# Ighina/MultimodalTopicSegmentation

Hardware: AMD Instinct MI355X
Metric: sentences/sec (fwd+bwd) (higher is better)
Workload: dtype bf16; 1 GPU; BASELINE configs[1]: restricted-window transformer tagger d=1792 heads=8 ff=256 radius=15 layers=1 focal loss, 64 docs x 256 sentences per GPU, fwd+bwd+Adam(eps 1e-7), inputs resident in HBM; global_batch_docs=64, sentences_per_doc=256, parallelism=dp1 (document-sharded, RCCL all-reduce)

## Files before the change

multimodaltopicsegmentation_amd/csrc/gemm.hip:

```cpp
#include <atomic>
#include <algorithm>
#include <math.h>
#include <stdlib.h>
#include "common.h"

#include "gemm_common.h"


template <int LAYOUT, typename TC, bool GLDS>
__global__ __launch_bounds__(256, 2) void gemm_bf16_kernel(const GemmArgs a) {
  constexpr bool A_KMAJOR = (LAYOUT == MTS_NT || LAYOUT == MTS_NN);
  constexpr bool B_KMAJOR = (LAYOUT == MTS_NT || LAYOUT == MTS_TT);
  extern __shared__ __attribute__((aligned(16))) char smem[];

  const int tid = threadIdx.x;
  const int lane = tid & 63;
  const int wave = tid >> 6;
  const int wm = wave >> 1, wn = wave & 1;
  const int r16 = lane & 15, g = lane >> 4;

  const int ntn = (a.N + BN - 1) / BN;
  const int ntm = (a.M + BM - 1) / BM;
  const int nt = ntn * ntm;
  int bid = blockIdx.x;
// ... 488 lines not shown
  const int m = (int)(idx / n4), n = 4 * (int)(idx % n4);
  float s[4] = {0.f, 0.f, 0.f, 0.f};
  if (accumulate) load4<float>(C + (size_t)m * ldc + n, s);
  const size_t plane = (size_t)M * N;
  for (int z = 0; z < splits; ++z) {
    float v[4];
    load4<float>(slab + z * plane + (size_t)m * N + n, v);
#pragma unroll
    for (int i = 0; i < 4; ++i) s[i] += v[i];
  }
  store4<float>(C + (size_t)m * ldc + n, s);
}

__global__ __launch_bounds__(256) void splitk_reduce_t_kernel(const float* __restrict__ slab, int splits, int M, int N, float* __restrict__ Ct,
                                                              int ldc, int accumulate) {
  __shared__ float tile[32][33];
  const int n0 = blockIdx.x * 32, m0 = blockIdx.y * 32;
  const int tx = threadIdx.x & 31, ty = threadIdx.x >> 5;
  const size_t plane = (size_t)M * N;
#pragma unroll
  for (int r = ty; r < 32; r += 8) {
    const int m = m0 + r, n = n0 + tx;
    float s = 0.f;
    if (m < M && n < N) {
      const float* p = slab + (size_t)m * N + n;
      int z = 0;
      for (; z + 7 < splits; z += 8) {
        float v[8];
#pragma unroll
        for (int u = 0; u < 8; ++u) v[u] = p[(size_t)(z + u) * plane];
#pragma unroll
        for (int u = 0; u < 8; ++u) s += v[u];
      }
      for (; z < splits; ++z) s += p[(size_t)z * plane];
    }
    tile[r][tx] = s;
  }
  __syncthreads();
#pragma unroll
  for (int r = ty; r < 32; r += 8) {
    const int n = n0 + r, m = m0 + tx;
    if (n < N && m < M) {
      float* o = Ct + (size_t)n * ldc + m;
      *o = accumulate ? *o + tile[tx][r] : tile[tx][r];
    }
  }
}

template <typename T> __global__ void cast_kernel(const float* __restrict__ src, T* __restrict__ dst, size_t n) {
  size_t i = ((size_t)blockIdx.x * blockDim.x + threadIdx.x) * 4;
  const size_t stride = (size_t)gridDim.x * blockDim.x * 4;
  for (; i + 3 < n; i += stride) {
    float v[4];
    load4<float>(src + i, v);
    store4<T>(dst + i, v);
  }
  if (i < n && i + 3 >= n)
    for (size_t j = i; j < n; ++j) dst[j] = from_f32<T>(src[j]);
}

template <typename T> __global__ void cast_concat_kernel(const float* __restrict__ s1, const float* __restrict__ s2, T* __restrict__ dst,
                                                          size_t rows, int D1, int D2) {
  const int D = D1 + D2, q = D / 4;
  const size_t total = rows * q;
  for (size_t i = (size_t)blockIdx.x * blockDim.x + threadIdx.x; i < total; i += (size_t)gridDim.x * blockDim.x) {
    const size_t r = i / q;
    const int e = (int)(i - r * q) * 4;
    float v[4];
    load4<float>(e < D1 ? s1 + r * D1 + e : s2 + r * D2 + (e - D1), v);
    store4<T>(dst + r * D + e, v);
  }
}

extern "C" int mts_cast_concat(void* stream, int dst_dtype, size_t rows, int D1, int D2, const float* src1, const float* src2, void* dst) {
  MTS_CHECK_ARG(src1 && src2 && dst && D1 > 0 && D2 > 0 && D1 % 4 == 0 && D2 % 4 == 0, "mts_cast_concat: bad arguments (widths must be multiples of 4)");
  if (rows == 0) return MTS_OK;
  const int blocks = (int)std::min<size_t>(4096, (rows * ((D1 + D2) / 4) + 255) / 256);
  if (dst_dtype == MTS_BF16) hipLaunchKernelGGL(cast_concat_kernel<bf16_t>, dim3(blocks), dim3(256), 0, (hipStream_t)stream, src1, src2, (bf16_t*)dst, rows, D1, D2);
  else if (dst_dtype == MTS_F32) hipLaunchKernelGGL(cast_concat_kernel<float>, dim3(blocks), dim3(256), 0, (hipStream_t)stream, src1, src2, (float*)dst, rows, D1, D2);
  else { mts_set_error("mts_cast_concat: bad dtype %d", dst_dtype); return MTS_ERR_INVALID; }
  MTS_LAUNCH_CHECK("mts_cast_concat");
  return MTS_OK;
}

extern "C" size_t mts_colsum_workspace(int N) { return (size_t)COLSUM_RS * (size_t)N * sizeof(float); }

extern "C" int mts_colsum(void* stream, int dtype, int M, int N, const void* X, int ldx, float* out, int accumulate,
                          void* partial) {
  MTS_CHECK_ARG(M > 0 && N > 0 && X && out && partial, "mts_colsum: bad arguments");
  MTS_CHECK_ARG(dtype == MTS_F32 || dtype == MTS_BF16, "mts_colsum: bad dtype %d", dtype);
  MTS_CHECK_ARG(ldx % 4 == 0, "mts_colsum: ldx must be a multiple of 4");
  hipStream_t st = (hipStream_t)stream;
  const int nparts = min(COLSUM_RS, M);
  dim3 grid(ceil_div(N, 64), COLSUM_RS);
  (void)nparts;
  if (dtype == MTS_F32)
    hipLaunchKernelGGL(colsum_partial_kernel<float>, grid, dim3(256), 0, st, (const float*)X, M, N, ldx, (float*)partial);
  else
    hipLaunchKernelGGL(colsum_partial_kernel<bf16_t>, grid, dim3(256), 0, st, (const bf16_t*)X, M, N, ldx, (float*)partial);
  hipLaunchKernelGGL(colsum_final_kernel, dim3(ceil_div(N, 64)), dim3(256), 0, st, (const float*)partial, N, COLSUM_RS, out,
                     accumulate);
  MTS_LAUNCH_CHECK("mts_colsum");
  return MTS_OK;
}

extern "C" int mts_cast(void* stream, int dst_dtype, const float* src, void* dst, size_t n) {
  MTS_CHECK_ARG(src && dst, "mts_cast: null pointer");
  if (n == 0) return MTS_OK;
  hipStream_t st = (hipStream_t)stream;
  const int blocks = (int)std::min<size_t>(2048, (n / 4 + 255) / 256 + 1);
  if (dst_dtype == MTS_BF16)
    hipLaunchKernelGGL(cast_kernel<bf16_t>, dim3(blocks), dim3(256), 0, st, src, (bf16_t*)dst, n);
  else if (dst_dtype == MTS_F32)
    hipLaunchKernelGGL(cast_kernel<float>, dim3(blocks), dim3(256), 0, st, src, (float*)dst, n);
  else {
    mts_set_error("mts_cast: bad dtype %d", dst_dtype);
    return MTS_ERR_INVALID;
  }
  MTS_LAUNCH_CHECK("mts_cast");
  return MTS_OK;
}

int mts_launch_gemm256(const GemmArgs& a, int layout, bool c_is_f32, int splits, hipStream_t st);
int mts_launch_gemm224(const GemmArgs& a, int layout, bool c_is_f32, int splits, hipStream_t st);
bool mts_gemm224t_applies(const GemmArgs& a, int layout, bool c_is_f32, int splits);

static thread_local int g_gemm_glds = -1;
static thread_local int g_tile_mode = -1;
static thread_local int g_force_splits = 0;
static thread_local int g_tile_order = 1;
static thread_local int g_gemm_deep = 1;
static thread_local int g_chain = 0;
static thread_local int g_combine = 0;
#define MTS_GEMM_WS_HEAD 8192
static thread_local int g_last_tile = 0, g_last_splits = 0;

static thread_local void (*g_mid_hook)(void) = nullptr;
extern "C" int mts_gemm_set_mid_hook(void (*fn)(void)) { g_mid_hook = fn; return MTS_OK; }

extern "C" int mts_gemm_last_plan(int* tile, int* splits) {
  if (tile) *tile = g_last_tile;
  if (splits) *splits = g_last_splits;
  return MTS_OK;
}

void mts_band_set_mfma(int on);
void mts_band_set_fused(int on);
static thread_local int g_f32_mfma = 1;
static thread_local int g_big_min_k = 256;
static thread_local int g_gemm_variant = 0;
void mts_lstm_pair_set_spin_limit(int n);
void mts_lstm_pair_set_max_pairs(int n);
void mts_lstm_pair_set_parts(int n);
extern "C" int mts_set_option(const char* key, int value) {
  if (!key) return MTS_ERR_INVALID;
  if (!strcmp(key, "gemm_tile")) { g_tile_mode = value; return MTS_OK; }
  if (!strcmp(key, "gemm_glds")) { g_gemm_glds = value; return MTS_OK; }
  if (!strcmp(key, "gemm_splits")) { g_force_splits = value; return MTS_OK; }
  if (!strcmp(key, "gemm_order")) { g_tile_order = value; return MTS_OK; }
  if (!strcmp(key, "gemm_chain")) { g_chain = value; return MTS_OK; }
  if (!strcmp(key, "gemm_combine")) { g_combine = value; return MTS_OK; }
  if (!strcmp(key, "gemm_deep")) { g_gemm_deep = value; return MTS_OK; }
  if (!strcmp(key, "gemm_variant")) { g_gemm_variant = value; return MTS_OK; }
  if (!strcmp(key, "gemm_big_min_k")) { g_big_min_k = value; return MTS_OK; }
  if (!strcmp(key, "gemm_f32_mfma")) { g_f32_mfma = value; return MTS_OK; }
  if (!strcmp(key, "band_mfma")) { mts_band_set_mfma(value); return MTS_OK; }
  if (!strcmp(key, "band_fused_bwd")) { mts_band_set_fused(value); return MTS_OK; }
  if (!strcmp(key, "lstm_pair_spin_limit")) { mts_lstm_pair_set_spin_limit(value); return MTS_OK; }
  if (!strcmp(key, "lstm_pair_max_pairs")) { mts_lstm_pair_set_max_pairs(value); return MTS_OK; }
  if (!strcmp(key, "lstm_parts")) { mts_lstm_pair_set_parts(value); return MTS_OK; }
  mts_set_error("mts_set_option: unknown key %s", key);
  return MTS_ERR_INVALID;
}

template <int LAYOUT, typename TC>
static void launch_bf16(const GemmArgs& a, int splits, hipStream_t st) {
  const int nt = ceil_div(a.M, BM) * ceil_div(a.N, BN);
  if (g_gemm_glds < 0) {
    const char* e = getenv("MTS_GEMM_GLDS");
    g_gemm_glds = (e && e[0] == '0') ? 0 : 1;
  }
  const bool glds = g_gemm_glds && (a.K % BK == 0) && (a.ksplit % BK == 0) && a.M >= 8 && a.N >= 8;
  if (glds) {
    GemmArgs b = a;
    const bool deep = g_gemm_deep && (size_t)nt * splits <= 256 && a.ksplit >= 4 * BK;
    b.nbuf = deep ? 4 : 2;
    auto k = gemm_bf16_kernel<LAYOUT, TC, true>;
    static std::atomic<bool> attr_set{false};
    if (deep && !attr_set.load(std::memory_order_acquire)) {
      if (hipFuncSetAttribute((const void*)k, hipFuncAttributeMaxDynamicSharedMemorySize, 8 * TILE_BYTES) != hipSuccess) b.nbuf = 2;
      else attr_set.store(true, std::memory_order_release);
    }
    hipLaunchKernelGGL(k, dim3(nt, 1, splits), dim3(256), (b.nbuf == 4 ? 8 : 4) * TILE_BYTES, st, b);
  } else {
    hipLaunchKernelGGL((gemm_bf16_kernel<LAYOUT, TC, false>), dim3(nt, 1, splits), dim3(256), 4 * TILE_BYTES, st, a);
  }
}

static void plan_bf16(int c_dtype, int layout, int M, int N, int K, unsigned epilogue, bool has_workspace, size_t workspace_bytes,
                      int* use256_out, int* splits_out) {
  if (g_tile_mode < 0) {
    const char* e = getenv("MTS_GEMM_TILE");
    g_tile_mode = e ? atoi(e) : 0;
  }
  const int tile_mode = g_tile_mode;
  const unsigned plain = epilogue & ~MTS_EPI_ACCUM;
  const bool can_split = (c_dtype == MTS_F32 && plain == 0 && has_workspace && N % 4 == 0 && K >= 2048);
  const bool can256 = (K % BK == 0) && K >= g_big_min_k && M >= 8 && N >= 8 && tile_mode != 128;
  const double bw = 3500.0;
  double best = 1e30;
  int splits = 1;
  int use256 = 0;
  const bool can224 = can256 && (N % 224 == 0) && tile_mode != 256;
  for (int big = 0; big <= (can256 ? 2 : 0); ++big) {
    if (big == 2 && !can224) continue;
    if (tile_mode == 256 && can256 && big != 1) continue;
    if (tile_mode == 224 && can224 && big != 2) continue;
    const int tile = big ? 256 : 128;
    const double slots = big ? 256.0 : 512.0;
    const double t_k = layout == MTS_TN ? (big == 2 ? (M % 256 == 0 ? 0.0160 : 0.0200) : big == 1 ? 0.0218 : 0.0145)
                                        : (big ? 0.0232 * (big == 2 ? 0.875 : 1.0) : 0.0180);
    const double t_0 = big ? 7.7 : 6.5;
    const int nt = ceil_div(M, tile) * (big == 2 ? N / 224 : ceil_div(N, tile));
    for (int sp = 1; sp <= (can_split ? 32 : 1); ++sp) {
      const int ks = ceil_div(ceil_div(K, sp), BK) * BK;
      if (ceil_div(K, ks) != sp) continue;
      if (sp > 1 && (size_t)sp * M * N * sizeof(float) > workspace_bytes) break;
      if (g_force_splits > 0 && can_split && sp != g_force_splits) continue;
      const double rounds = ceil((double)nt * sp / slots);
      const double cost = rounds * (ks * t_k + t_0) + (sp > 1 ? (2.0 * sp + 1.0) * M * N * 4.0 / 1e6 / bw : 0.0);
      if (cost < best) { best = cost; splits = sp; use256 = big; }
    }
  }
  *use256_out = use256;
  *splits_out = splits;
}

int mts_gemm224_last_kernel();
int mts_launch_gemm224t_pair(const GemmArgs& a, int splits, const void* A2, const void* B2, float* slab2, hipStream_t st);
bool mts_gemm224t_applies(const GemmArgs& a, int layout, bool c_is_f32, int splits);

static int wgrad_pair_splits(int M, int N, int K, size_t workspace_bytes) {
  if (M % 256 || N % 224 || K % 64 || K < 256) return -1;
  static int cus = 0;
  if (!cus) { int dev = 0; hipDeviceProp_t pr; cus = (hipGetDevice(&dev) == hipSuccess && hipGetDeviceProperties(&pr, dev) == hipSuccess) ? pr.multiProcessorCount : 256; }
  const int nt = (M / 256) * (N / 224);
  int sp = std::max(1, std::min(32, cus / (2 * nt)));
  for (; sp >= 1; --sp) {
    const int ks = ceil_div(ceil_div(K, sp), BK) * BK;
    if (ceil_div(K, ks) != sp) continue;
    if (ks >= 128 && K - (sp - 1) * ks >= 128 && (size_t)2 * sp * M * N * sizeof(float) <= workspace_bytes) return sp;
  }
  return -1;
}
extern "C" size_t mts_wgrad_pair_workspace(int M, int N, int K) {
  const int sp = wgrad_pair_splits(M, N, K, (size_t)-1);
  return sp < 1 ? 0 : (size_t)2 * sp * M * N * sizeof(float);
}
extern "C" int mts_wgrad_pair(void* stream, int M, int N, int K, const void* A1, const void* B1, float* C1, int ldc1, const void* A2, const void* B2,
                              float* C2t, int ldc2t, int lda, int ldb, int accumulate, void* workspace, size_t workspace_bytes) {
  MTS_CHECK_ARG(M > 0 && N > 0 && K > 0 && A1 && B1 && C1 && A2 && B2 && C2t && workspace, "mts_wgrad_pair: bad arguments");
  MTS_CHECK_ARG(ldc1 >= N && ldc2t >= M && ldc1 % 4 == 0, "mts_wgrad_pair: bad output strides");
  const int sp = wgrad_pair_splits(M, N, K, workspace_bytes);
  MTS_UNSUPPORTED(sp >= 1, "mts_wgrad_pair: M=%d N=%d K=%d not covered (M %% 256, N %% 224, K %% 64) or workspace too small", M, N, K);
  hipStream_t st = (hipStream_t)stream;
  GemmArgs a;
  memset(&a, 0, sizeof(a));
  a.A = A1; a.B = B1; a.C = C1;
  a.M = M; a.N = N; a.K = K; a.lda = lda; a.ldb = ldb; a.ldc = ldc1;
  a.epi = 0; a.colscale = 1.0f;
  a.ksplit = ceil_div(ceil_div(K, sp), BK) * BK;
  a.order = 1; a.nbuf = 2; a.variant = 0;
  float* const planes = (float*)workspace;
  a.slab = planes;
  float* const planes2 = planes + (size_t)sp * M * N;
  MTS_UNSUPPORTED(mts_gemm224t_applies(a, MTS_TN, true, sp), "mts_wgrad_pair: operands not covered by the four-wave weight-gradient kernel (alignment / strides)");
  const int rc = mts_launch_gemm224t_pair(a, sp, A2, B2, planes2, st);
  MTS_UNSUPPORTED(rc == MTS_OK, "mts_wgrad_pair: launch refused");
  hipLaunchKernelGGL(splitk_reduce_kernel, dim3((unsigned)(((size_t)M * (N / 4) + 255) / 256)), dim3(256), 0, st, (const float*)planes, sp, M, N, C1, ldc1,
                     accumulate ? 1 : 0);
  hipLaunchKernelGGL(splitk_reduce_t_kernel, dim3(ceil_div(N, 32), ceil_div(M, 32)), dim3(256), 0, st, (const float*)planes2, sp, M, N, C2t, ldc2t,
                     accumulate ? 1 : 0);
  MTS_LAUNCH_CHECK("mts_wgrad_pair");
  return MTS_OK;
}

extern "C" int mts_gemm_plan(int a_dtype, int c_dtype, int layout, int M, int N, int K, unsigned epilogue, size_t workspace_bytes,
                             int* tile, int* splits) {
  MTS_CHECK_ARG(M > 0 && N > 0 && K > 0, "mts_gemm_plan: bad shape M=%d N=%d K=%d", M, N, K);
  MTS_CHECK_ARG(layout == MTS_NT || layout == MTS_NN || layout == MTS_TN || layout == MTS_TT, "mts_gemm_plan: bad layout %d", layout);
  MTS_CHECK_ARG(a_dtype == MTS_F32 || a_dtype == MTS_BF16, "mts_gemm_plan: bad a_dtype %d", a_dtype);
  int use256 = 0, sp = 1;
  const size_t ws_planes = workspace_bytes > MTS_GEMM_WS_HEAD ? workspace_bytes - MTS_GEMM_WS_HEAD : 0;
  if (a_dtype == MTS_BF16) plan_bf16(c_dtype, layout, M, N, K, epilogue, ws_planes > 0, ws_planes, &use256, &sp);
  if (tile) *tile = a_dtype == MTS_F32 ? (g_f32_mfma ? 128 : 64) : use256 == 2 ? 224 : use256 == 1 ? 256 : 128;
  if (splits) *splits = sp;
  return MTS_OK;
}

extern "C" int mts_gemm(void* stream, int a_dtype, int c_dtype, int layout, int M, int N, int K, const void* A, int lda,
                        const void* B, int ldb, void* C, int ldc, const float* bias, const void* residual, int ldr,
                        void* aux, int ldaux, unsigned epilogue, float colscale, int ncols_scaled, void* workspace, size_t workspace_bytes) {
  MTS_CHECK_ARG(M > 0 && N > 0 && K > 0, "mts_gemm: bad shape M=%d N=%d K=%d", M, N, K);
  MTS_CHECK_ARG(A && B && C, "mts_gemm: null operand");
  MTS_CHECK_ARG(layout == MTS_NT || layout == MTS_NN || layout == MTS_TN || layout == MTS_TT, "mts_gemm: bad layout %d", layout);
  MTS_CHECK_ARG(a_dtype == MTS_F32 || a_dtype == MTS_BF16, "mts_gemm: bad a_dtype %d", a_dtype);
  MTS_CHECK_ARG(c_dtype == MTS_F32 || c_dtype == a_dtype, "mts_gemm: c_dtype must be f32 or a_dtype");
  MTS_CHECK_ARG(!(epilogue & MTS_EPI_BIAS) || bias, "mts_gemm: MTS_EPI_BIAS without bias");
  MTS_CHECK_ARG(!(epilogue & MTS_EPI_RESIDUAL) || residual, "mts_gemm: MTS_EPI_RESIDUAL without residual");
  MTS_CHECK_ARG(!(epilogue & MTS_EPI_ACCUM) || c_dtype == MTS_F32, "mts_gemm: MTS_EPI_ACCUM needs fp32 C");
  MTS_CHECK_ARG((epilogue & (MTS_EPI_GELU | MTS_EPI_RELU)) != (MTS_EPI_GELU | MTS_EPI_RELU), "mts_gemm: MTS_EPI_GELU and MTS_EPI_RELU are exclusive");
  hipStream_t st = (hipStream_t)stream;
  GemmArgs a;
  a.A = A; a.B = B; a.C = C; a.bias = bias; a.residual = residual; a.aux = aux;
  a.M = M; a.N = N; a.K = K; a.lda = lda; a.ldb = ldb; a.ldc = ldc; a.ldr = ldr; a.ldaux = ldaux;
  a.epi = epilogue; a.colscale = colscale; a.ncols_scaled = ncols_scaled;
  a.variant = g_gemm_variant;
#ifdef MTS_GEMM_STAMPS
  a.stamps = nullptr;
#endif
  a.ksplit = K; a.slab = nullptr; a.chain = nullptr; a.order = g_tile_order; a.nbuf = 2;

  if (a_dtype == MTS_F32) {
// ... 87 lines not shown
```

multimodaltopicsegmentation_amd/csrc/norm.hip:

```cpp
#include <algorithm>
#include <type_traits>
#include "common.h"
#include "loss_elems.h"

#define ROW_WAVES 4
#define BWD_MAX_BLOCKS 512

template <typename T, int NV> struct RowRegs {
  float v[NV][4];
  __device__ __forceinline__ void load(const T* row, int D, int lane) {
#pragma unroll
    for (int i = 0; i < NV; ++i) {
      const int e = 4 * (lane + 64 * i);
      if (e < D) load4<T>(row + e, v[i]);
      else { v[i][0] = v[i][1] = v[i][2] = v[i][3] = 0.f; }
    }
  }
  __device__ __forceinline__ void store(T* row, int D, int lane) const {
#pragma unroll
    for (int i = 0; i < NV; ++i) {
      const int e = 4 * (lane + 64 * i);
      if (e < D) store4<T>(row + e, v[i]);
    }
  }
  __device__ __forceinline__ void zero() {
#pragma unroll
    for (int i = 0; i < NV; ++i) v[i][0] = v[i][1] = v[i][2] = v[i][3] = 0.f;
  }
};

template <int NV> __device__ __forceinline__ void row_stats(const float (&x)[NV][4], int D, int lane, float& mean, float& rstd, float eps) {
  float s = 0.f;
#pragma unroll
  for (int i = 0; i < NV; ++i) s += (x[i][0] + x[i][1]) + (x[i][2] + x[i][3]);
  mean = wave_sum(s) / (float)D;
  float q = 0.f;
#pragma unroll
  for (int i = 0; i < NV; ++i) {
    if (4 * (lane + 64 * i) < D) {
#pragma unroll
      for (int j = 0; j < 4; ++j) { const float d = x[i][j] - mean; q += d * d; }
    }
  }
  rstd = 1.0f / sqrtf(wave_sum(q) / (float)D + eps);
}

template <typename T, int NV, int EMBED, bool FULL = false>
__global__ __launch_bounds__(64 * ROW_WAVES) void ln_fwd_kernel(
    const void* __restrict__ xin, const float* __restrict__ pos, int pos_offset, int L, const float* __restrict__ type0,
    const float* __restrict__ gamma, const float* __restrict__ beta, float eps, int rows, int D,
    T* __restrict__ y, T* __restrict__ pre, float* __restrict__ mean_out, float* __restrict__ rstd_out,
    const float* __restrict__ head_w, const float* __restrict__ head_b, int n_out, float* __restrict__ scores,
    const int32_t* __restrict__ row_src, const float* __restrict__ xin2 = nullptr, int D1 = 0) {
  const int lane = threadIdx.x & 63;
  const int row = blockIdx.x * ROW_WAVES + (threadIdx.x >> 6);
  if (row >= rows) return;
  float gv[NV][4], bv[NV][4];
#pragma unroll
  for (int i = 0; i < NV; ++i) {
    const int e = 4 * (lane + 64 * i);
    if (FULL || e < D) { load4<float>(gamma + e, gv[i]); load4<float>(beta + e, bv[i]); }
  }
  float x[NV][4];
  if constexpr (EMBED) {
    const int src = row_src ? row_src[row] : row;
    const int Dx = xin2 ? D1 : D;
    const float* xr = reinterpret_cast<const float*>(xin) + (size_t)src * Dx;
    const float* xr2 = xin2 ? xin2 + (size_t)src * (D - D1) - D1 : xr;
    const float* pr = pos + (size_t)(pos_offset + src % L) * D;
#pragma unroll
    for (int i = 0; i < NV; ++i) {
      const int e = 4 * (lane + 64 * i);
      if (FULL || e < D) {
        float a[4], b[4], c[4];
        if constexpr (EMBED == 2) load4<bf16_t>(reinterpret_cast<const bf16_t*>(xin) + (size_t)src * D + e, a);
        else load4<float>((e < Dx ? xr : xr2) + e, a);
        load4<float>(pr + e, b); load4<float>(type0 + e, c);
#pragma unroll
        for (int j = 0; j < 4; ++j) x[i][j] = (a[j] + b[j]) + c[j];
        if constexpr (sizeof(T) == 2) {
#pragma unroll
          for (int j = 0; j < 4; ++j) x[i][j] = to_f32(from_f32<T>(x[i][j]));
        }
      } else { x[i][0] = x[i][1] = x[i][2] = x[i][3] = 0.f; }
    }
    if (pre) {
#pragma unroll
      for (int i = 0; i < NV; ++i) { const int e = 4 * (lane + 64 * i); if (FULL || e < D) store4<T>(pre + (size_t)row * D + e, x[i]); }
    }
  } else {
    const T* xr = reinterpret_cast<const T*>(xin) + (size_t)row * D;
#pragma unroll
    for (int i = 0; i < NV; ++i) {
      const int e = 4 * (lane + 64 * i);
      if (FULL || e < D) load4<T>(xr + e, x[i]);
      else { x[i][0] = x[i][1] = x[i][2] = x[i][3] = 0.f; }
    }
  }
  float mean, rstd;
  row_stats<NV>(x, D, lane, mean, rstd, eps);
  float hs[4] = {0.f, 0.f, 0.f, 0.f};
  const float* hwp = head_w ? head_w : gamma;
  const int hw_max = head_w ? n_out - 1 : 0;
#pragma unroll
  for (int i = 0; i < NV; ++i) {
    const int e = 4 * (lane + 64 * i);
    if (FULL || e < D) {
#pragma unroll
      for (int j = 0; j < 4; ++j) x[i][j] = (x[i][j] - mean) * rstd * gv[i][j] + bv[i][j];
      if (head_w) {
#pragma unroll
        for (int c = 0; c < 4; ++c) {
          float w[4];
          load4<float>(hwp + (size_t)min(c, hw_max) * D + e, w);
#pragma unroll
          for (int j = 0; j < 4; ++j) hs[c] += to_f32(from_f32<T>(x[i][j])) * w[j];
        }
      }
    }
  }
  if (y) {
#pragma unroll
    for (int i = 0; i < NV; ++i) {
      const int e = 4 * (lane + 64 * i);
      if (FULL || e < D) store4<T>(y + (size_t)row * D + e, x[i]);
    }
  }
  if (lane == 0 && mean_out) { mean_out[row] = mean; rstd_out[row] = rstd; }
  if (head_w) {
    for (int c = 0; c < n_out; ++c) {
      const float s = wave_sum(hs[c]);
      if (lane == 0) scores[(size_t)row * n_out + c] = s + head_b[c];
    }
  }
}

template <typename T>
__global__ __launch_bounds__(64 * ROW_WAVES) void head_fwd_kernel(const T* __restrict__ x, int ldx, int rows, int D, int n_out,
                                                                const float* __restrict__ w, const float* __restrict__ b,
                                                                float* __restrict__ scores) {
  const int lane = threadIdx.x & 63;
  const int row = blockIdx.x * ROW_WAVES + (threadIdx.x >> 6);
  if (row >= rows) return;
  float hs[4] = {0.f, 0.f, 0.f, 0.f};
  for (int e = 4 * lane; e < D; e += 256) {
    float xv[4];
    load4<T>(x + (size_t)row * ldx + e, xv);
    for (int c = 0; c < n_out; ++c) {
      float wv[4];
      load4<float>(w + (size_t)c * D + e, wv);
#pragma unroll
      for (int j = 0; j < 4; ++j) hs[c] += xv[j] * wv[j];
    }
  }
  for (int c = 0; c < n_out; ++c) {
    const float s = wave_sum(hs[c]);
    if (lane == 0) scores[(size_t)row * n_out + c] = s + b[c];
  }
}

template <typename T>
__global__ __launch_bounds__(256) void head_bwd_data_kernel(const float* __restrict__ ds, const float* __restrict__ w, int rows, int D,
                                                            int n_out, T* __restrict__ dx, int lddx, int accumulate) {
  const size_t idx = (size_t)blockIdx.x * 256 + threadIdx.x;
  const int per_row = D / 4;
  const size_t total = (size_t)rows * per_row;
  if (idx >= total) return;
  const int row = (int)(idx / per_row);
  const int e = 4 * (int)(idx % per_row);
  float o[4] = {0.f, 0.f, 0.f, 0.f};
  if (accumulate) load4<T>(dx + (size_t)row * lddx + e, o);
  for (int c = 0; c < n_out; ++c) {
    const float s = ds[(size_t)row * n_out + c];
    float wv[4];
    load4<float>(w + (size_t)c * D + e, wv);
#pragma unroll
    for (int j = 0; j < 4; ++j) o[j] += s * wv[j];
  }
  store4<T>(dx + (size_t)row * lddx + e, o);
}

struct EmbArgs { int B, L, Bc, nchunks; const int32_t* row0; const int32_t* lengths; float* dpos_part; };

template <typename T, int NV, bool WIDE, bool FULL = false, int NHG = 0, bool EMB = false>
__global__ __launch_bounds__(64 * ROW_WAVES, 2) void ln_bwd_kernel(
    const T* __restrict__ x, const T* __restrict__ dy_, const float* __restrict__ dlogit, const float* __restrict__ head_w, int n_out,
    const float* __restrict__ gamma, const float* __restrict__ mean, const float* __restrict__ rstd, int rows, int D,
    T* __restrict__ dx, float* __restrict__ partial, const EmbArgs ea) {
  static_assert(!(EMB && (WIDE || NHG > 0)), "the embedding form has no head and D <= 2048");
  constexpr bool HG = NHG > 0;
  constexpr int NR = HG ? NHG + 1 : EMB ? 2 : 3;
  constexpr int NS = HG ? NHG + 2 : NR;
  constexpr int NA = HG ? NHG : 2;
  const T* __restrict__ dy = HG ? nullptr : dy_;
  __shared__ float red[ROW_WAVES][NR][64 * 4];
  __shared__ __attribute__((aligned(16))) float gam_s[NV * 256];
  __shared__ __attribute__((aligned(16))) float hw_s[EMB ? 1 : 4][EMB ? 4 : NV * 256];
  __shared__ __attribute__((aligned(16))) float task_s[EMB ? ROW_WAVES : 1][EMB ? NV * 256 : 4];
  const int lane = threadIdx.x & 63;
  const int wave = __builtin_amdgcn_readfirstlane(threadIdx.x >> 6);
  const int col0 = WIDE ? (int)blockIdx.y * (NV * 256) : 0;
  for (int idx = threadIdx.x; idx < NV * 256; idx += 64 * ROW_WAVES) {
    const int e = col0 + idx;
    gam_s[idx] = (e < D) ? gamma[e] : 0.f;
    if constexpr (!EMB) {
      if (head_w)
// ... 626 lines not shown
      for (int c = 0; c < 4; ++c)
#pragma unroll
        for (int j = 0; j < 4; ++j) dw[c][i][j] += dl[c] * xv[i][j];
  }
  float* slab = partial + (size_t)blockIdx.x * 5 * D;
#pragma unroll
  for (int i = 0; i < NV; ++i) {
    __syncthreads();
#pragma unroll
    for (int c = 0; c < 4; ++c)
#pragma unroll
      for (int j = 0; j < 4; ++j) red[wave][c][lane * 4 + j] = dw[c][i][j];
    __syncthreads();
    for (int t = threadIdx.x; t < 4 * 256; t += 64 * ROW_WAVES) {
      const int slot = t / 256, col = t % 256;
      const int e = col0 + 256 * i + col;
      if (e < D) {
        float s = 0.f;
#pragma unroll
        for (int w = 0; w < ROW_WAVES; ++w) s += red[w][slot][col];
        slab[(size_t)slot * D + e] = s;
      }
    }
  }
  __syncthreads();
  if (lane == 0)
    for (int c = 0; c < 4; ++c) red[wave][c][0] = dbs[c];
  __syncthreads();
  if (threadIdx.x < 4) {
    float s = 0.f;
    for (int w = 0; w < ROW_WAVES; ++w) s += red[w][threadIdx.x][0];
    slab[(size_t)4 * D + threadIdx.x] = s;
  }
}

#define SR_COLS 32
struct SlabOuts { float* o[6]; int short_slot, short_len; const float* alt; int alt_slot, alt_nb; };
__global__ __launch_bounds__(256) void slab_reduce_kernel(const float* __restrict__ partial, int nblocks, int nslots, int D, const SlabOuts so) {
  __shared__ float4 red[32][8];
  const int c4 = threadIdx.x & 7, grp = threadIdx.x >> 3;
  const int e = blockIdx.x * SR_COLS + 4 * c4;
  const int slot = blockIdx.y;
  float* o = so.o[slot];
  if (!o) return;
  if (slot == so.alt_slot) { partial = so.alt - (size_t)slot * D; nblocks = so.alt_nb; nslots = 1; }
  const int len = (slot == so.short_slot) ? so.short_len : D;
  float4 s = make_float4(0.f, 0.f, 0.f, 0.f);
  if (e < len) {
    const float* p = partial + (size_t)slot * D + e;
    const size_t bs = (size_t)nslots * D;
    int b = grp;
    for (; b + 32 * 7 < nblocks; b += 32 * 8) {
      float4 v[8];
#pragma unroll
      for (int u = 0; u < 8; ++u) v[u] = *reinterpret_cast<const float4*>(p + (size_t)(b + 32 * u) * bs);
#pragma unroll
      for (int u = 0; u < 8; ++u) { s.x += v[u].x; s.y += v[u].y; s.z += v[u].z; s.w += v[u].w; }
    }
    for (; b < nblocks; b += 32) {
      const float4 v = *reinterpret_cast<const float4*>(p + (size_t)b * bs);
      s.x += v.x; s.y += v.y; s.z += v.z; s.w += v.w;
    }
  }
  red[grp][c4] = s;
  __syncthreads();
  if (grp == 0 && e < len) {
    float4 t = red[0][c4];
#pragma unroll
    for (int gidx = 1; gidx < 32; ++gidx) { const float4 v = red[gidx][c4]; t.x += v.x; t.y += v.y; t.z += v.z; t.w += v.w; }
    if (e + 3 < len) *reinterpret_cast<float4*>(o + e) = t;
    else { const float tv[4] = {t.x, t.y, t.z, t.w}; for (int j = 0; j < 4 && e + j < len; ++j) o[e + j] = tv[j]; }
  }
}

int mts_slab_reduce_rows(hipStream_t st, const float* partial, int nblocks, int D, float* out) {
  SlabOuts so = {{out, nullptr, nullptr, nullptr, nullptr, nullptr}, -1, 0, nullptr, -1, 0};
  hipLaunchKernelGGL(slab_reduce_kernel, dim3(ceil_div(D, SR_COLS), 1), dim3(256), 0, st, partial, nblocks, 1, D, so);
  MTS_LAUNCH_CHECK("slab_reduce");
  return MTS_OK;
}

template <typename T>
__global__ __launch_bounds__(256) void embed_bwd_kernel(const T* __restrict__ dpre, int B, int L, int D, float* __restrict__ dpos, int pos_offset,
                                                        const int32_t* __restrict__ row0, const int32_t* __restrict__ lengths) {
  const size_t idx = (size_t)blockIdx.x * 256 + threadIdx.x;
  const int per_row = D / 4;
  if (idx >= (size_t)L * per_row) return;
  const int i = (int)(idx / per_row), e = 4 * (int)(idx % per_row);
  float s[4] = {0.f, 0.f, 0.f, 0.f};
  int b = 0;
  if (row0) {
    for (; b < B; ++b) {
      if (i < lengths[b]) {
        float v[4];
        load4<T>(dpre + ((size_t)row0[b] + i) * D + e, v);
#pragma unroll
        for (int j = 0; j < 4; ++j) s[j] += v[j];
      }
    }
  }
  for (; b + 7 < B; b += 8) {
    float v[8][4];
#pragma unroll
    for (int u = 0; u < 8; ++u) load4<T>(dpre + ((size_t)(b + u) * L + i) * D + e, v[u]);
#pragma unroll
    for (int u = 0; u < 8; ++u)
#pragma unroll
      for (int j = 0; j < 4; ++j) s[j] += v[u][j];
  }
  for (; b < B; ++b) {
    float v[4];
    load4<T>(dpre + ((size_t)b * L + i) * D + e, v);
#pragma unroll
    for (int j = 0; j < 4; ++j) s[j] += v[j];
  }
  float* o = dpos + (size_t)(pos_offset + i) * D + e;
  float cur[4];
  load4<float>(o, cur);
#pragma unroll
  for (int j = 0; j < 4; ++j) cur[j] += s[j];
  store4<float>(o, cur);
}
static inline int pick_nv(int D) {
  const int need = ceil_div(D, 256);
  if (need <= 1) return 1;
  if (need <= 2) return 2;
  if (need <= 4) return 4;
  if (need == 7) return 7;
  if (need <= 8) return 8;
  if (need <= 16) return 16;
  return 0;
}

template <typename F> static inline void dispatch_nv(int nv, F&& f) {
  switch (nv) {
    case 1: f(std::integral_constant<int, 1>{}); break;
    case 2: f(std::integral_constant<int, 2>{}); break;
    case 4: f(std::integral_constant<int, 4>{}); break;
    case 7: f(std::integral_constant<int, 7>{}); break;
    case 8: f(std::integral_constant<int, 8>{}); break;
    default: f(std::integral_constant<int, 16>{}); break;
  }
}
template <typename F> static inline void dispatch_nv8(int nv, F&& f) {
  switch (nv) {
    case 1: f(std::integral_constant<int, 1>{}); break;
    case 2: f(std::integral_constant<int, 2>{}); break;
    case 4: f(std::integral_constant<int, 4>{}); break;
    case 7: f(std::integral_constant<int, 7>{}); break;
    default: f(std::integral_constant<int, 8>{}); break;
  }
}

template <typename T, int EMBED>
static int ln_fwd_launch(hipStream_t st, const void* x, const float* pos, int pos_offset, int L, const float* type0, const float* gamma,
                         const float* beta, float eps, int rows, int D, void* y, void* pre, float* mean, float* rstd,
                         const float* head_w, const float* head_b, int n_out, float* scores, const int32_t* row_src = nullptr,
                         const float* x2 = nullptr, int D1 = 0) {
  const int nv = pick_nv(D);
  MTS_UNSUPPORTED(nv > 0 && D % 4 == 0, "layernorm: D=%d must be a multiple of 4 and <= 4096", D);
  dim3 grid(ceil_div(rows, ROW_WAVES)), block(64 * ROW_WAVES);
  dispatch_nv(nv, [&](auto nvc) {
    constexpr int NV = decltype(nvc)::value;
    if (D == NV * 256)
      hipLaunchKernelGGL((ln_fwd_kernel<T, NV, EMBED, true>), grid, block, 0, st, x, pos, pos_offset, L, type0, gamma, beta, eps, rows, D, (T*)y,
                         (T*)pre, mean, rstd, head_w, head_b, n_out, scores, row_src, x2, D1);
    else
      hipLaunchKernelGGL((ln_fwd_kernel<T, NV, EMBED>), grid, block, 0, st, x, pos, pos_offset, L, type0, gamma, beta, eps, rows, D, (T*)y,
                         (T*)pre, mean, rstd, head_w, head_b, n_out, scores, row_src, x2, D1);
  });
  MTS_LAUNCH_CHECK("layernorm_fwd");
  return MTS_OK;
}

static int embed_ln_fwd(void* stream, int dtype, int B, int L, int D, const float* x, const float* x2, int D1, const float* pos, int pos_offset,
                        const float* type0, const float* gamma, const float* beta, float eps, void* y, void* pre, float* mean, float* rstd,
                        const int32_t* row_src, int n_rows, const char* who) {
  MTS_CHECK_ARG(B > 0 && L > 0 && D > 0 && x && pos && type0 && gamma && beta && y, "%s: bad arguments", who);
  MTS_CHECK_ARG(!row_src || (n_rows > 0 && n_rows <= B * L), "%s: packed form needs 0 < n_rows <= B*L", who);
  MTS_CHECK_ARG(!x2 || (D1 > 0 && D1 < D && D1 % 4 == 0), "%s: the first part's width must be a multiple of 4 inside (0, D)", who);
  const int rows = row_src ? n_rows : B * L;
  if (dtype == MTS_F32)
    return ln_fwd_launch<float, 1>((hipStream_t)stream, x, pos, pos_offset, L, type0, gamma, beta, eps, rows, D, y, pre, mean, rstd,
                                      nullptr, nullptr, 0, nullptr, row_src, x2, D1);
  if (dtype == MTS_BF16)
    return ln_fwd_launch<bf16_t, 1>((hipStream_t)stream, x, pos, pos_offset, L, type0, gamma, beta, eps, rows, D, y, pre, mean, rstd,
                                       nullptr, nullptr, 0, nullptr, row_src, x2, D1);
  mts_set_error("%s: bad dtype %d", who, dtype);
  return MTS_ERR_INVALID;
}

extern "C" int mts_embed_layernorm_fwd(void* stream, int dtype, int B, int L, int D, const float* x, const float* pos, int pos_offset,
                                       const float* type0, const float* gamma, const float* beta, float eps, void* y, void* pre,
                                       float* mean, float* rstd, const int32_t* row_src, int n_rows) {
  return embed_ln_fwd(stream, dtype, B, L, D, x, nullptr, 0, pos, pos_offset, type0, gamma, beta, eps, y, pre, mean, rstd, row_src, n_rows,
                      "mts_embed_layernorm_fwd");
}

extern "C" int mts_embed_layernorm_fwd_x16(void* stream, int B, int L, int D, const void* x_bf16, const float* pos, int pos_offset, const float* type0,
                                           const float* gamma, const float* beta, float eps, void* y, void* pre, float* mean, float* rstd,
                                           const int32_t* row_src, int n_rows) {
  MTS_CHECK_ARG(B > 0 && L > 0 && D > 0 && x_bf16 && pos && type0 && gamma && beta && y, "mts_embed_layernorm_fwd_x16: bad arguments");
  MTS_CHECK_ARG(!row_src || (n_rows > 0 && n_rows <= B * L), "mts_embed_layernorm_fwd_x16: packed form needs 0 < n_rows <= B*L");
  MTS_CHECK_ARG(((uintptr_t)x_bf16 & 7) == 0, "mts_embed_layernorm_fwd_x16: x must be 8-byte aligned");
  const int rows = row_src ? n_rows : B * L;
  return ln_fwd_launch<bf16_t, 2>((hipStream_t)stream, x_bf16, pos, pos_offset, L, type0, gamma, beta, eps, rows, D, y, pre, mean, rstd, nullptr, nullptr, 0,
                                  nullptr, row_src, nullptr, 0);
}

extern "C" int mts_embed_layernorm_fwd2(void* stream, int dtype, int B, int L, int D1, int D2, const float* x1, const float* x2, const float* pos,
                                        int pos_offset, const float* type0, const float* gamma, const float* beta, float eps, void* y, void* pre,
                                        float* mean, float* rstd, const int32_t* row_src, int n_rows) {
  MTS_CHECK_ARG(x2 && D2 > 0 && D2 % 4 == 0, "mts_embed_layernorm_fwd2: second part missing or its width not a multiple of 4");
  return embed_ln_fwd(stream, dtype, B, L, D1 + D2, x1, x2, D1, pos, pos_offset, type0, gamma, beta, eps, y, pre, mean, rstd, row_src, n_rows,
                      "mts_embed_layernorm_fwd2");
}

extern "C" int mts_layernorm_fwd(void* stream, int dtype, int rows, int D, const void* x, const float* gamma, const float* beta, float eps,
                                 void* y, float* mean, float* rstd, const float* head_w, const float* head_b, int n_out, float* scores) {
  MTS_CHECK_ARG(rows > 0 && D > 0 && x && gamma && beta && (y || (head_w && mean && rstd)), "mts_layernorm_fwd: bad arguments (y may be NULL only with a fused head and saved statistics)");
  MTS_CHECK_ARG(!head_w || (head_b && scores && n_out >= 1 && n_out <= 4), "mts_layernorm_fwd: fused head needs head_b, scores, n_out<=4");
  if (dtype == MTS_F32)
    return ln_fwd_launch<float, 0>((hipStream_t)stream, x, nullptr, 0, 1, nullptr, gamma, beta, eps, rows, D, y, nullptr, mean, rstd,
                                       head_w, head_b, n_out, scores);
  if (dtype == MTS_BF16)
    return ln_fwd_launch<bf16_t, 0>((hipStream_t)stream, x, nullptr, 0, 1, nullptr, gamma, beta, eps, rows, D, y, nullptr, mean, rstd,
                                        head_w, head_b, n_out, scores);
  mts_set_error("mts_layernorm_fwd: bad dtype %d", dtype);
  return MTS_ERR_INVALID;
}

extern "C" size_t mts_layernorm_bwd_workspace(int D) { return (size_t)BWD_MAX_BLOCKS * 6 * (size_t)D * sizeof(float); }

template <typename T>
static int ln_bwd_launch(hipStream_t st, int rows, int D, const void* x, const void* dy, const float* dlogit, const float* head_w, int n_out,
                         const float* gamma, const float* beta, const float* mean, const float* rstd, void* dx, float* dgamma, float* dbeta,
                         float* dxsum, float* dhead_w, float* dhead_b, void* partial) {
  const int nv = pick_nv(D);
  MTS_UNSUPPORTED(nv > 0 && D % 4 == 0, "layernorm_bwd: D=%d must be a multiple of 4 and <= 4096", D);
  const int blocks = std::min(BWD_MAX_BLOCKS, ceil_div(rows, ROW_WAVES));
  const int nhg = dhead_w ? n_out : 0;
  const EmbArgs ea = {0, 0, 0, 0, nullptr, nullptr, nullptr};
  auto go = [&](auto k, dim3 grid) {
    hipLaunchKernelGGL(k, grid, dim3(64 * ROW_WAVES), 0, st, (const T*)x, (const T*)dy, dlogit, head_w, n_out, gamma, mean, rstd, rows, D,
                       (T*)dx, (float*)partial, ea);
  };
  if (nv <= 8) {
    dispatch_nv8(nv, [&](auto nvc) {
      constexpr int NV = decltype(nvc)::value;
      if (D == NV * 256) {
        if (nhg == 1) go(ln_bwd_kernel<T, NV, false, true, 1>, dim3(blocks));
        else if (nhg == 2) go(ln_bwd_kernel<T, NV, false, true, 2>, dim3(blocks));
        else go(ln_bwd_kernel<T, NV, false, true>, dim3(blocks));
      } else {
        if (nhg == 1) go(ln_bwd_kernel<T, NV, false, false, 1>, dim3(blocks));
        else if (nhg == 2) go(ln_bwd_kernel<T, NV, false, false, 2>, dim3(blocks));
        else go(ln_bwd_kernel<T, NV, false>, dim3(blocks));
      }
    });
  } else {
    if (nhg == 1) go(ln_bwd_kernel<T, 8, true, false, 1>, dim3(blocks, ceil_div(D, 2048)));
    else if (nhg == 2) go(ln_bwd_kernel<T, 8, true, false, 2>, dim3(blocks, ceil_div(D, 2048)));
    else go(ln_bwd_kernel<T, 8, true>, dim3(blocks, ceil_div(D, 2048)));
  }
  if (nhg == 1)
    hipLaunchKernelGGL(ln_head_final_kernel<1>, dim3(ceil_div(D, 32)), dim3(256), 0, st, (const float*)partial, blocks, D, head_w, gamma, beta, dgamma,
                       dbeta, dxsum, dhead_w, dhead_b, (const float*)nullptr, (float*)nullptr);
  else if (nhg == 2)
    hipLaunchKernelGGL(ln_head_final_kernel<2>, dim3(ceil_div(D, 32)), dim3(256), 0, st, (const float*)partial, blocks, D, head_w, gamma, beta, dgamma,
                       dbeta, dxsum, dhead_w, dhead_b, (const float*)nullptr, (float*)nullptr);
  else {
    SlabOuts so = {{dgamma, dbeta, dxsum, nullptr, nullptr, nullptr}, -1, 0, nullptr, -1, 0};
    hipLaunchKernelGGL(slab_reduce_kernel, dim3(ceil_div(D, SR_COLS), 3), dim3(256), 0, st, (const float*)partial, blocks, 3, D, so);
  }
  MTS_LAUNCH_CHECK("layernorm_bwd");
  return MTS_OK;
}

extern "C" int mts_layernorm_bwd(void* stream, int dtype, int rows, int D, const void* x, const void* dy, const float* dlogit,
                                 const float* head_w, int n_out, const float* gamma, const float* mean, const float* rstd, void* dx,
                                 float* dgamma, float* dbeta, float* dxsum, void* partial, const float* beta, float* dhead_w, float* dhead_b) {
  MTS_CHECK_ARG(rows > 0 && D > 0 && x && gamma && mean && rstd && dx && partial, "mts_layernorm_bwd: bad arguments");
  MTS_CHECK_ARG(dy || head_w, "mts_layernorm_bwd: needs dy and/or a fused head gradient");
  MTS_CHECK_ARG(!head_w || (dlogit && n_out >= 1 && n_out <= 4), "mts_layernorm_bwd: fused head needs dlogit, n_out<=4");
  MTS_CHECK_ARG(!dhead_w || (head_w && beta && dhead_b && n_out <= 2 && !dy),
                "mts_layernorm_bwd: head parameter gradients need head_w, beta, dhead_b, n_out <= 2 and dy == NULL (the last layer)");
  if (dtype == MTS_F32)
    return ln_bwd_launch<float>((hipStream_t)stream, rows, D, x, dy, dlogit, head_w, n_out, gamma, beta, mean, rstd, dx, dgamma, dbeta, dxsum, dhead_w, dhead_b, partial);
  if (dtype == MTS_BF16)
    return ln_bwd_launch<bf16_t>((hipStream_t)stream, rows, D, x, dy, dlogit, head_w, n_out, gamma, beta, mean, rstd, dx, dgamma, dbeta, dxsum, dhead_w, dhead_b, partial);
  mts_set_error("mts_layernorm_bwd: bad dtype %d", dtype);
  return MTS_ERR_INVALID;
}

extern "C" int mts_layernorm_loss_tail_supported(int dtype, int D, int n_out) {
  return (dtype == MTS_F32 || dtype == MTS_BF16) && (n_out == 1 || n_out == 2) && D % 256 == 0 &&
         (D == 256 || D == 512 || D == 1024 || D == 1792 || D == 2048);
}

template <typename T>
static int ln_tail_launch(hipStream_t st, int rows, int D, const void* x, const float* gamma, const float* beta, float eps, const float* head_w,
                          const float* head_b, int n_out, void* dx, float* dgamma, float* dbeta, float* dxsum, float* dhead_w, float* dhead_b,
                          float* ws, const TailArgs& ta0) {
  const int nv = D / 256;
  const int blocks = std::min(BWD_MAX_BLOCKS, ceil_div(rows, ROW_WAVES));
  TailArgs ta = ta0;
  ta.loss_part = ws + (size_t)BWD_MAX_BLOCKS * 5 * D;
  dispatch_nv8(nv, [&](auto nvc) {
    constexpr int NV = decltype(nvc)::value;
    if (n_out == 1)
      hipLaunchKernelGGL((ln_tail_kernel<T, NV, 1>), dim3(blocks), dim3(64 * ROW_WAVES), 0, st, (const T*)x, gamma, beta, eps, head_w, head_b, rows, D, (T*)dx, ws, ta);
    else
      hipLaunchKernelGGL((ln_tail_kernel<T, NV, 2>), dim3(blocks), dim3(64 * ROW_WAVES), 0, st, (const T*)x, gamma, beta, eps, head_w, head_b, rows, D, (T*)dx, ws, ta);
  });
// ... 205 lines not shown
```

Baseline: 9.227 million sentences/s.

## Add persistent grid-stride LayerNorm forward with LDS-cached params and row prefetch

Adds a persistent variant of the LayerNorm forward kernel. Each wave walks several rows with a grid stride and prefetches the next row's inputs while it normalizes the current one. Gamma, beta, type0 and the head weights are staged once per block in LDS instead of being reloaded by every wave. The grid is capped to occupancy times CU count, and the path is on by default for D<=2048 without a second input. It aims to cut repeated parameter loads and hide memory latency, at the cost of dynamic LDS use, extra registers and fewer blocks.

```diff
diff --git a/multimodaltopicsegmentation_amd/csrc/gemm.hip b/multimodaltopicsegmentation_amd/csrc/gemm.hip
--- a/multimodaltopicsegmentation_amd/csrc/gemm.hip
+++ b/multimodaltopicsegmentation_amd/csrc/gemm.hip
@@ -664,6 +664,7 @@
 void mts_lstm_pair_set_spin_limit(int n);
 void mts_lstm_pair_set_max_pairs(int n);
 void mts_lstm_pair_set_parts(int n);
+void mts_ln_set_fwd_rows_per_wave(int r);
 extern "C" int mts_set_option(const char* key, int value) {
   if (!key) return MTS_ERR_INVALID;
   if (!strcmp(key, "gemm_tile")) { g_tile_mode = value; return MTS_OK; }
@@ -681,6 +682,7 @@
   if (!strcmp(key, "lstm_pair_spin_limit")) { mts_lstm_pair_set_spin_limit(value); return MTS_OK; }
   if (!strcmp(key, "lstm_pair_max_pairs")) { mts_lstm_pair_set_max_pairs(value); return MTS_OK; }
   if (!strcmp(key, "lstm_parts")) { mts_lstm_pair_set_parts(value); return MTS_OK; }
+  if (!strcmp(key, "ln_fwd_rows_per_wave")) { mts_ln_set_fwd_rows_per_wave(value); return MTS_OK; }
   mts_set_error("mts_set_option: unknown key %s", key);
   return MTS_ERR_INVALID;
 }
diff --git a/multimodaltopicsegmentation_amd/csrc/norm.hip b/multimodaltopicsegmentation_amd/csrc/norm.hip
--- a/multimodaltopicsegmentation_amd/csrc/norm.hip
+++ b/multimodaltopicsegmentation_amd/csrc/norm.hip
@@ -45,13 +45,162 @@
   rstd = 1.0f / sqrtf(wave_sum(q) / (float)D + eps);
 }
 
-template <typename T, int NV, int EMBED, bool FULL = false>
+template <typename T, int NV, int EMBED, bool FULL>
+__device__ __forceinline__ void ln_fwd_walk(
+    const void* __restrict__ xin, const float* __restrict__ pos, int pos_offset, int L, const float* __restrict__ type0,
+    const float* __restrict__ gamma, const float* __restrict__ beta, float eps, int rows, int D,
+    T* __restrict__ y, T* __restrict__ pre, float* __restrict__ mean_out, float* __restrict__ rstd_out,
+    const float* __restrict__ head_w, const float* __restrict__ head_b, int n_out, float* __restrict__ scores,
+    const int32_t* __restrict__ row_src, const float* __restrict__ xin2, int D1) {
+  constexpr int W = NV * 256;
+  extern __shared__ __attribute__((aligned(16))) float ln_lds[];
+  float* gam_s = ln_lds;
+  float* bet_s = gam_s + W;
+  float* t0_s = bet_s + W;
+  float* hw_s = t0_s + (EMBED ? W : 0);
+  const int lane = threadIdx.x & 63;
+  const int wave = __builtin_amdgcn_readfirstlane(threadIdx.x >> 6);
+  if constexpr (EMBED != 0) head_w = nullptr;
+  const int hw_max = head_w ? n_out - 1 : 0;
+  for (int idx = threadIdx.x; idx < W; idx += 64 * ROW_WAVES) {
+    const bool in = idx < D;
+    gam_s[idx] = in ? gamma[idx] : 0.f;
+    bet_s[idx] = in ? beta[idx] : 0.f;
+    if constexpr (EMBED != 0) t0_s[idx] = in ? type0[idx] : 0.f;
+    if (head_w)
+      for (int c = 0; c < n_out; ++c) hw_s[c * W + idx] = in ? head_w[(size_t)c * D + idx] : 0.f;
+  }
+  float hb[4] = {0.f, 0.f, 0.f, 0.f};
+  if (head_w) {
+#pragma unroll
+    for (int c = 0; c < 4; ++c) hb[c] = head_b[min(c, hw_max)];
+  }
+  __syncthreads();
+  const int stride = gridDim.x * ROW_WAVES;
+  int row = blockIdx.x * ROW_WAVES + wave;
+  if (row >= rows) return;
+  using XT = std::conditional_t<EMBED == 0, T, std::conditional_t<EMBED == 2, bf16_t, float>>;
+  Pack<XT, 4> px[NV];
+  Pack<float, 4> pp[EMBED ? NV : 1];
+  auto fetch = [&](int r, int src) {
+    if constexpr (EMBED) {
+      const XT* xr = reinterpret_cast<const XT*>(xin) + (size_t)src * D;
+      const float* pr = pos + (size_t)(pos_offset + src % L) * D;
+#pragma unroll
+      for (int i = 0; i < NV; ++i) {
+        const int e = 4 * (lane + 64 * i);
+        if (FULL || e < D) { px[i].load(xr + e); pp[i].load(pr + e); }
+      }
+    } else {
+      const T* xr = reinterpret_cast<const T*>(xin) + (size_t)r * D;
+#pragma unroll
+      for (int i = 0; i < NV; ++i) {
+        const int e = 4 * (lane + 64 * i);
+        if (FULL || e < D) px[i].load(xr + e);
+      }
+    }
+  };
+  float x[NV][4];
+  auto consume = [&]() {
+    int lo = 4 * lane;
+    asm volatile("" : "+v"(lo));
+#pragma unroll
+    for (int i = 0; i < NV; ++i) {
+      const int e = 4 * (lane + 64 * i);
+      if (FULL || e < D) {
+        if constexpr (EMBED) {
+          const float4 c4 = *reinterpret_cast<const float4*>(t0_s + lo + 256 * i);
+          const float c[4] = {c4.x, c4.y, c4.z, c4.w};
+#pragma unroll
+          for (int j = 0; j < 4; ++j) x[i][j] = (px[i].get(j) + pp[i].get(j)) + c[j];
+          if constexpr (sizeof(T) == 2) {
+#pragma unroll
+            for (int j = 0; j < 4; ++j) x[i][j] = to_f32(from_f32<T>(x[i][j]));
+          }
+        } else {
+#pragma unroll
+          for (int j = 0; j < 4; ++j) x[i][j] = px[i].get(j);
+        }
+      } else { x[i][0] = x[i][1] = x[i][2] = x[i][3] = 0.f; }
+      asm volatile("" : "+v"(x[i][0]), "+v"(x[i][1]), "+v"(x[i][2]), "+v"(x[i][3]) : : "memory");
+    }
+  };
+  int src = (EMBED && row_src) ? row_src[row] : row;
+  fetch(row, src);
+  int src_n = row + stride;
+  if (EMBED && row_src && src_n < rows) src_n = row_src[src_n];
+  consume();
+  while (true) {
+    int lo = 4 * lane;
+    asm volatile("" : "+v"(lo));
+    const int nrow = row + stride;
+    if (nrow < rows) {
+      fetch(nrow, src_n);
+      if (EMBED && row_src && nrow + stride < rows) src_n = row_src[nrow + stride];
+      else src_n = nrow + stride;
+    }
+    if constexpr (EMBED) {
+      if (pre) {
+#pragma unroll
+        for (int i = 0; i < NV; ++i) { const int e = 4 * (lane + 64 * i); if (FULL || e < D) store4<T>(pre + (size_t)row * D + e, x[i]); }
+      }
+    }
+    float mean, rstd;
+    row_stats<NV>(x, D, lane, mean, rstd, eps);
+    float hs[4] = {0.f, 0.f, 0.f, 0.f};
+#pragma unroll
+    for (int i = 0; i < NV; ++i) {
+      const int e = 4 * (lane + 64 * i);
+      if (FULL || e < D) {
+        const float4 g4 = *reinterpret_cast<const float4*>(gam_s + lo + 256 * i);
+        const float4 b4 = *reinterpret_cast<const float4*>(bet_s + lo + 256 * i);
+        const float gv[4] = {g4.x, g4.y, g4.z, g4.w}, bv[4] = {b4.x, b4.y, b4.z, b4.w};
+#pragma unroll
+        for (int j = 0; j < 4; ++j) x[i][j] = (x[i][j] - mean) * rstd * gv[j] + bv[j];
+        if (head_w) {
+#pragma unroll
+          for (int c = 0; c < 4; ++c) {
+            const float4 w4 = *reinterpret_cast<const float4*>(hw_s + min(c, hw_max) * W + lo + 256 * i);
+            const float w[4] = {w4.x, w4.y, w4.z, w4.w};
+#pragma unroll
+            for (int j = 0; j < 4; ++j) hs[c] += to_f32(from_f32<T>(x[i][j])) * w[j];
+          }
+        }
+      }
+    }
+#pragma unroll
+    for (int i = 0; i < NV; ++i) {
+      const int e = 4 * (lane + 64 * i);
+      if (FULL || e < D) store4<T>(y + (size_t)row * D + e, x[i]);
+    }
+    if (lane == 0 && mean_out) { mean_out[row] = mean; rstd_out[row] = rstd; }
+    if (head_w) {
+#pragma unroll
+      for (int c = 0; c < 4; ++c) {
+        if (c < n_out) {
+          const float s = wave_sum(hs[c]);
+          if (lane == 0) scores[(size_t)row * n_out + c] = s + hb[c];
+        }
+      }
+    }
+    if (nrow >= rows) break;
+    row = nrow;
+    consume();
+  }
+}
+
+template <typename T, int NV, int EMBED, bool FULL = false, bool WALK = false>
 __global__ __launch_bounds__(64 * ROW_WAVES) void ln_fwd_kernel(
     const void* __restrict__ xin, const float* __restrict__ pos, int pos_offset, int L, const float* __restrict__ type0,
     const float* __restrict__ gamma, const float* __restrict__ beta, float eps, int rows, int D,
     T* __restrict__ y, T* __restrict__ pre, float* __restrict__ mean_out, float* __restrict__ rstd_out,
     const float* __restrict__ head_w, const float* __restrict__ head_b, int n_out, float* __restrict__ scores,
     const int32_t* __restrict__ row_src, const float* __restrict__ xin2 = nullptr, int D1 = 0) {
+  if constexpr (WALK) {
+    ln_fwd_walk<T, NV, EMBED, FULL>(xin, pos, pos_offset, L, type0, gamma, beta, eps, rows, D, y, pre, mean_out, rstd_out, head_w, head_b,
+                                    n_out, scores, row_src, xin2, D1);
+    return;
+  }
   const int lane = threadIdx.x & 63;
   const int row = blockIdx.x * ROW_WAVES + (threadIdx.x >> 6);
   if (row >= rows) return;
@@ -984,6 +1133,15 @@
   }
 }
 
+static thread_local int g_ln_fwd_rpw = 0;
+void mts_ln_set_fwd_rows_per_wave(int r) { g_ln_fwd_rpw = std::max(0, r); }
+
+static int num_cus() {
+  static int cus = 0;
+  if (!cus) { int dev = 0; hipDeviceProp_t pr; cus = (hipGetDevice(&dev) == hipSuccess && hipGetDeviceProperties(&pr, dev) == hipSuccess) ? pr.multiProcessorCount : 256; }
+  return cus;
+}
+
 template <typename T, int EMBED>
 static int ln_fwd_launch(hipStream_t st, const void* x, const float* pos, int pos_offset, int L, const float* type0, const float* gamma,
                          const float* beta, float eps, int rows, int D, void* y, void* pre, float* mean, float* rstd,
@@ -992,6 +1150,27 @@
   const int nv = pick_nv(D);
   MTS_UNSUPPORTED(nv > 0 && D % 4 == 0, "layernorm: D=%d must be a multiple of 4 and <= 4096", D);
   dim3 grid(ceil_div(rows, ROW_WAVES)), block(64 * ROW_WAVES);
+  if (g_ln_fwd_rpw != 1 && nv <= 8 && y && !x2) {
+    const size_t lds = (size_t)(2 + (EMBED ? 1 : 0) + (head_w ? n_out : 0)) * nv * 256 * sizeof(float);
+    dispatch_nv8(nv, [&](auto nvc) {
+      constexpr int NV = decltype(nvc)::value;
+      auto go = [&](auto k) {
+        int blocks = g_ln_fwd_rpw > 1 ? ceil_div(rows, ROW_WAVES * g_ln_fwd_rpw) : ceil_div(rows, ROW_WAVES);
+        if (g_ln_fwd_rpw == 0) {
+          static int per_cu[5] = {};
+          int& pc = per_cu[head_w ? n_out : 0];
+          if (!pc && hipOccupancyMaxActiveBlocksPerMultiprocessor(&pc, (const void*)k, 64 * ROW_WAVES, lds) != hipSuccess) pc = 1;
+          blocks = std::min(blocks, std::max(1, pc) * num_cus());
+        }
+        hipLaunchKernelGGL(k, dim3(blocks), block, lds, st, x, pos, pos_offset, L, type0, gamma, beta, eps, rows, D, (T*)y, (T*)pre, mean, rstd,
+                           head_w, head_b, n_out, scores, row_src, x2, D1);
+      };
+      if (D == NV * 256) go(ln_fwd_kernel<T, NV, EMBED, true, true>);
+      else go(ln_fwd_kernel<T, NV, EMBED, false, true>);
+    });
+    MTS_LAUNCH_CHECK("layernorm_fwd");
+    return MTS_OK;
+  }
   dispatch_nv(nv, [&](auto nvc) {
     constexpr int NV = decltype(nvc)::value;
     if (D == NV * 256)
```

New measurement: 9.284 million sentences/s (median of 6 runs). About the same (+0.6%).
